# GATB/MindTheGap

Measured on AMD Instinct MI355X. Metric: breakpoints filled/sec, higher is better.
Workload: dtype u64; 1 GPU; synthetic human-scale: 3 Gbp i.i.d. donor as 600000 x 5 kb sequences, 100000 insertion sites (50-1000 nt) per batch, k=31, max-nodes 100; sites_per_batch=100000, sites_per_rank_and_step=100000, distinct_batches_per_rank=4, site_set=400000, donor_sequences=600000, erroneous_fragments=0, k=31, max_nodes=100, max_length=10000, nb_solid_kmers=3108581096, nb_unitigs=600024, index_bytes=60154587216, unitig_store_bytes=3945966160, batches_in_flight=6, input=prepared batches, resident in HBM, output=C-ABI records + ASCII sequences in page-locked host memory

## Files before the change

### mindthegap_amd/csrc/mtg_gpu_fill.hip

```cpp
#include "mtg_gpu_common.h"

namespace mtgi {

enum { TRAVERSAL_SETS = mtg_index::NWS };
__constant__ Index c_ix[TRAVERSAL_SETS];
__constant__ FillCfg c_cfg[TRAVERSAL_SETS];

#ifndef MTG_STAGE_A_WAVES
#define MTG_STAGE_A_WAVES 2
#endif
#ifndef MTG_WALK_WAVES
#define MTG_WALK_WAVES 2
#endif
enum { PARK_LISTS = 19 };
struct ParkCtl {
    uint32_t count[PARK_LISTS];
    uint32_t n_branching;
    uint32_t pad_[3];
#ifdef MTG_BUBBLE_TIMING
    uint32_t hist_lane[32], hist_wave[32], hist_walk_lane[32], hist_walk_wave[32];
#endif
};
#ifdef MTG_BUBBLE_TIMING
__device__ __forceinline__ void timing_note(uint32_t* hl, uint32_t* hw, uint64_t t0)
// ... 950 lines not shown
            const uint32_t general_hint = ws.post_general == ~0u ? m : (uint32_t)std::min<uint64_t>(m, 4ull * ws.post_general + 1024ull);
            hipLaunchKernelGGL(k_post, dim3(general_hint), dim3(64), 0, stream, idx->dev, cfg, d_raw.as<uint8_t>(), d_head.as<uint8_t>(), d_out.as<GapOut>(), ids, d_tle, d_tbad, d_toff, d_tcnt, d_mis, d_fok,
                               in.want_all_contigs ? 1u : 0u, d_rec.as<SlotRec>(), m, park, (const uint32_t*)d_pi_head, (const uint32_t*)d_pi_next, pi_mask, d_rw, d_roff, d_tie_p);
            hipLaunchKernelGGL(k_post_lean, dim3((m + 64 / POST_LEAN_G - 1) / (64 / POST_LEAN_G)), dim3(64), 0, stream, idx->dev, cfg, d_raw.as<uint8_t>(), d_head.as<uint8_t>(), d_out.as<GapOut>(), in.want_all_contigs ? 1u : 0u, d_rec.as<SlotRec>(), m);
            const ScanBegin sbegin{{0, 0, arena_used[0], arena_used[1]}};
            hipLaunchKernelGGL(k_scan1, dim3(nblocks), dim3(SCAN_SL), 0, stream, d_rec.as<SlotRec>(), m, d_blocks.as<ScanBlock>());
            hipLaunchKernelGGL(k_scan2, dim3(1), dim3(256), 0, stream, d_blocks.as<ScanBlock>(), nblocks, sbegin, d_tot.as<PartTot>(), h_tot, park);
            HIP_TRY(hipGetLastError());
            EmitDev D;
            EmitHost H;
            const double share = std::min(1.0, std::max(0.0, tune::f(tune::T_PACKED_SEQ_SHARE, 0.0)));
            const uint32_t pack_q = (uint32_t)std::lround(share * 65536.0);
            bool packed = want_records && combo && identity && arena_used[0] == 0 && pack_q != 0;
            uint64_t shadow_halves = 0;
            if (packed) {
                shadow_halves = 2 * ((((uint64_t)sink.seq_cap * pack_q) >> 16) / 32 + 3);
                HIP_TRY(d_shadow.alloc(shadow_halves * 4));
            }
            auto emit = [&]() -> int {
                D.seq = sink.seq_dev ? sink.seq_dev : p_seq(); D.ext = d_ext.as<char>();
                D.seq_cap = sink.seq_cap; D.ext_cap = sink.ext_cap;
                D.res = p_res(); D.fil = p_fil();
                D.dense_words = d_dw.as<uint64_t>(); D.dense_meta = d_dm.as<uint32_t>();
                D.dense_cap_words = ws.cap[d_dw.slot] / 8; D.dense_cap_contigs = ws.cap[d_dm.slot] / 20;
                const bool want_wire = sink.wire_dev != nullptr && identity && tier == 0;
                D.wire = want_wire ? (uint8_t*)sink.wire_dev : nullptr; D.wire_cap = sink.wire_cap; D.wire_tag = sink.wire_tag;
                D.tot = d_tot.as<PartTot>(); D.wire_gaps = m;
                D.shadow = packed ? d_shadow.as<uint32_t>() : nullptr; D.shadow_cap = shadow_halves; D.pack_q = pack_q;
                if (packed) HIP_TRY(hipMemsetAsync(d_shadow.p, 0, shadow_halves * 4, stream));
                if (want_wire) HIP_TRY(hipMemsetAsync(sink.wire_dev, 0, sizeof(mtg_wire_header), stream));
                H.seq = sink.seq; H.ext = sink.ext; H.fil = sink.fil;
                if (!want_wire)
                    hipLaunchKernelGGL(k_emit_lean, dim3((m + 64 / EMIT_LEAN_G - 1) / (64 / EMIT_LEAN_G)), dim3(64), 0, stream, idx->dev.us, cfg, d_raw.as<uint8_t>(), d_head.as<uint8_t>(), d_rec.as<SlotRec>(), d_blocks.as<ScanBlock>(),
                                       ids, d_flags, k, D, H, m);
                hipLaunchKernelGGL(k_emit, dim3(want_wire ? m : general_hint), dim3(64), 0, stream, idx->dev.us, cfg, d_raw.as<uint8_t>(), d_head.as<uint8_t>(), d_rec.as<SlotRec>(), d_blocks.as<ScanBlock>(), ids, d_flags, k, D, H,
                                   d_rlist.as<uint32_t>(), d_glist.as<uint32_t>(), m, park, want_wire ? 0u : 1u);
                if (want_wire) hipLaunchKernelGGL(k_wire_sum, dim3(256 * 4), dim3(256), 0, stream, (uint8_t*)sink.wire_dev, sink.wire_cap);
                HIP_TRY(hipGetLastError());
                return MTG_OK;
            };
            HIP_TRY(mark(eve));
            if (int erc = emit()) return erc;
            HIP_TRY(hipEventRecord(ev2, stream));
            tick("host prep+launch");
            if (while_busy && !busy_done) { busy_done = true; (*while_busy)(); tick("host work during kernels"); }
            HIP_TRY(hipEventSynchronize(ev2));
            traversal_lock.unlock();
            tick("totals ready");
            t0 = now_ms();
            PartTot tot = *h_tot;
            const uint64_t need_w = tot.end[0] * 8 + 64, need_m = tot.end[1] * 20 + 64;
            bool again = false;
            if (want_records && tot.end[2] > sink.seq_cap) {
                const uintptr_t old = (uintptr_t)sink.seq, old_end = old + sink.seq_cap;
                const uintptr_t old_fil = (uintptr_t)sink.fil, old_fil_end = old_fil + n * sizeof(mtg_filled);
                if (!sink.grow_seq || !sink.grow_seq((size_t)tot.end[2], (size_t)tot.begin[2])) { set_error("sequence buffer too small: %llu bytes needed", (unsigned long long)tot.end[2]); return MTG_ERR_ARG; }
                if (launches > 1 && (uintptr_t)sink.seq != old)
                    for (size_t i = 0; i < n; i++) { const uintptr_t q = (uintptr_t)sink.fil[i].seq; if (q >= old && q < old_end) sink.fil[i].seq = sink.seq + (q - old); }
                if (launches > 1 && (uintptr_t)sink.fil != old_fil)
                    for (size_t i = 0; i < n; i++) { const uintptr_t q = (uintptr_t)sink.res[i].filled; if (q >= old_fil && q < old_fil_end) sink.res[i].filled = (const mtg_filled*)((const char*)sink.fil + (q - old_fil)); }
                again = true;
            }
            if (want_records && tot.end[3] > sink.ext_cap) {
                const uintptr_t old = (uintptr_t)sink.ext, old_end = old + sink.ext_cap;
                if (!sink.grow_ext || !sink.grow_ext((size_t)tot.end[3], (size_t)tot.begin[3])) { set_error("extension buffer too small: %llu bytes needed", (unsigned long long)tot.end[3]); return MTG_ERR_NOMEM; }
                if (launches > 1 && (uintptr_t)sink.ext != old)
                    for (size_t i = 0; i < n; i++) { const uintptr_t q = (uintptr_t)sink.res[i].extension; if (q >= old && q < old_end) sink.res[i].extension = sink.ext + (q - old); }
                again = true;
            }
            if (need_w > ws.cap[d_dw.slot] || need_m > ws.cap[d_dm.slot]) again = true;
            if (again) {
                HIP_TRY(hipStreamSynchronize(stream));
                if (combo) HIP_TRY(d_combo.grow_keeping(sink.combo_off_seq + std::max<size_t>(sink.seq_cap, 64) + SEQ_SLACK, sink.combo_off_seq + (size_t)tot.begin[2]));
                else if (!sink.seq_dev) HIP_TRY(d_seq.grow_keeping(std::max<size_t>(sink.seq_cap, 64) + SEQ_SLACK, (size_t)tot.begin[2]));
                HIP_TRY(d_ext.alloc(std::max<size_t>(sink.ext_cap, 64)));
                HIP_TRY(d_dw.alloc(need_w));
                HIP_TRY(d_dm.alloc(need_m));
                hipLaunchKernelGGL(k_scan1, dim3(nblocks), dim3(SCAN_SL), 0, stream, d_rec.as<SlotRec>(), m, d_blocks.as<ScanBlock>());
                hipLaunchKernelGGL(k_scan2, dim3(1), dim3(256), 0, stream, d_blocks.as<ScanBlock>(), nblocks, sbegin, d_tot.as<PartTot>(), (PartTot*)nullptr, park);
                packed = false;
                if (int erc = emit()) return erc;
            }
            CopyTurn copy_turn(idx->device);
            std::vector<mtg_gap_result> tmp_res;
            std::vector<mtg_filled> tmp_fil;
            const bool one_copy = combo && identity && tot.begin[2] == 0;
            const uint64_t pack_x = packed ? packed_split(tot.end[2], pack_q) : 0, pack_words = packed ? (tot.end[2] - pack_x + 31) / 32 : 0;
            uint64_t* h_shadow = nullptr;
            if (packed) {
                h_shadow = (uint64_t*)staging_host(&ws, Workspace::NHOST - 3, pack_words * 8 + 64);
                if (!h_shadow) { set_error("no page-locked memory for the packed sequences of a launch"); return MTG_ERR_NOMEM; }
            }
            if (want_records) {
                if (h_shadow) {
                    HIP_TRY(hipMemcpyAsync(sink.combo, d_combo.p, sink.combo_off_seq, hipMemcpyDeviceToHost, stream));
                    if (pack_words) HIP_TRY(hipMemcpyAsync(h_shadow, d_shadow.p, pack_words * 8, hipMemcpyDeviceToHost, stream));
                    HIP_TRY(hipEventRecord(evp, stream));
                    if (pack_x) HIP_TRY(hipMemcpyAsync(sink.combo + sink.combo_off_seq, (const char*)d_combo.p + sink.combo_off_seq, pack_x, hipMemcpyDeviceToHost, stream));
                } else if (one_copy) HIP_TRY(hipMemcpyAsync(sink.combo, d_combo.p, sink.combo_off_seq + (size_t)tot.end[2], hipMemcpyDeviceToHost, stream));
                else if (identity) {
                    HIP_TRY(hipMemcpyAsync(sink.res, p_res(), (size_t)m * sizeof(mtg_gap_result), hipMemcpyDeviceToHost, stream));
                    HIP_TRY(hipMemcpyAsync(sink.fil, p_fil(), (size_t)m * sizeof(mtg_filled), hipMemcpyDeviceToHost, stream));
                } else {
                    tmp_res.resize(m);
                    tmp_fil.resize(m);
                    HIP_TRY(hipMemcpyAsync(tmp_res.data(), p_res(), (size_t)m * sizeof(mtg_gap_result), hipMemcpyDeviceToHost, stream));
                    HIP_TRY(hipMemcpyAsync(tmp_fil.data(), p_fil(), (size_t)m * sizeof(mtg_filled), hipMemcpyDeviceToHost, stream));
                }
                const WireLayout wl = wire_layout(m, tot.n_filled, tot.end[2], tot.end[3]);
                const bool wired = sink.wire_dev != nullptr && identity && tier == 0 && wl.total <= sink.wire_cap && tot.n_retry == 0 && tot.n_general == 0;
                if (sink.wire_dev && identity && tier == 0) { sink.wire_ok = wired; sink.wire_bytes = wired ? wl.total : 0; }
                const char* seq_src = wired ? (const char*)sink.wire_dev + wl.o_seq : (sink.seq_dev ? sink.seq_dev : p_seq());
                if (!one_copy && !sink.seq_on_device && !sink.seq_stays_in_workspace && tot.end[2] > tot.begin[2]) HIP_TRY(hipMemcpyAsync(sink.seq + tot.begin[2], seq_src + tot.begin[2], tot.end[2] - tot.begin[2], hipMemcpyDeviceToHost, stream));
                if (tot.end[3] > tot.begin[3]) HIP_TRY(hipMemcpyAsync(sink.ext + tot.begin[3], d_ext.as<char>() + tot.begin[3], tot.end[3] - tot.begin[3], hipMemcpyDeviceToHost, stream));
            }
            std::vector<uint32_t> rlist(tot.n_retry), glist(tot.n_general);
            const bool dev_general = tot.n_general > 0 && !host_paths && !in.want_all_contigs && !tune::on(tune::T_HOST_GENERAL) && !tl_host_general;
            GenCtl* h_gctl = nullptr;
            GenDev GD{};
            if (dev_general) {
                const uint64_t ng = tot.n_general;
                HIP_TRY(d_paths.alloc(ng * (size_t)PATHS_WORDS * 4));
                HIP_TRY(d_ggaps.alloc(ng * sizeof(GenGap) + sizeof(GenCtl)));
                GD.cap_sols = 4 * ng + 1024; GD.cap_ascii = ng * 1280 + (1u << 20); GD.cap_tmp = ng * 48 + (1u << 17); GD.cap_bnd = 1u << 22;
                HIP_TRY(d_gsols.alloc(GD.cap_sols * sizeof(GenSol)));
                HIP_TRY(d_gascii.alloc(GD.cap_ascii + 64));
                HIP_TRY(d_gtmp.alloc(GD.cap_tmp * 8));
                HIP_TRY(d_gbnd.alloc(GD.cap_bnd * sizeof(NwCell)));
                GD.ctl = (GenCtl*)d_ggaps.p;
                GD.gaps = (GenGap*)((char*)d_ggaps.p + sizeof(GenCtl));
                GD.sols = d_gsols.as<GenSol>(); GD.ascii = d_gascii.as<char>(); GD.tmp = d_gtmp.as<uint64_t>(); GD.bnd = d_gbnd.as<NwCell>();
                HIP_TRY(hipMemsetAsync(GD.ctl, 0, sizeof(GenCtl), stream));
                hipLaunchKernelGGL(k_paths, dim3((unsigned)ng), dim3(64), 0, stream, cfg, d_raw.as<uint8_t>(), d_head.as<uint8_t>(), d_out.as<GapOut>(), d_glist.as<uint32_t>(), k, d_paths.as<uint32_t>(), (uint32_t)ng);
                hipLaunchKernelGGL(k_general, dim3((unsigned)ng), dim3(64), 0, stream, idx->dev, cfg, d_raw.as<uint8_t>(), d_head.as<uint8_t>(), d_out.as<GapOut>(), d_glist.as<uint32_t>(), ids, d_paths.as<uint32_t>(),
                                   d_tcnt, d_fok, d_src, d_flags, k, GD, (uint32_t)ng);
                HIP_TRY(hipGetLastError());
                h_gctl = (GenCtl*)staging_host(&ws, Workspace::NHOST - 2, sizeof(GenCtl) + ng * sizeof(GenGap) + 64);
                if (!h_gctl) { set_error("no page-locked memory for the multi-contig gaps of a launch"); return MTG_ERR_NOMEM; }
                HIP_TRY(hipMemcpyAsync(h_gctl, d_ggaps.p, sizeof(GenCtl) + ng * sizeof(GenGap), hipMemcpyDeviceToHost, stream));
            }
            HostChunk* hc = nullptr;
            SlotRec* h_rec = nullptr;
            uint64_t* h_w = nullptr;
            uint32_t* h_m = nullptr;
            const uint64_t tw = tot.end[0], tc = tot.end[1];
            if (tot.n_retry) HIP_TRY(hipMemcpyAsync(rlist.data(), d_rlist.p, (size_t)tot.n_retry * 4, hipMemcpyDeviceToHost, stream));
            auto contigs_to_host = [&]() -> int {
                hc->carve(m, tw, tc, h_rec, h_w, h_m);
                HIP_TRY(hipMemcpyAsync(h_rec, d_rec.p, (size_t)m * sizeof(SlotRec), hipMemcpyDeviceToHost, stream));
                if (tw) HIP_TRY(hipMemcpyAsync(h_w, d_dw.p, tw * 8, hipMemcpyDeviceToHost, stream));
                if (tc) HIP_TRY(hipMemcpyAsync(h_m, d_dm.p, tc * 20, hipMemcpyDeviceToHost, stream));
                return MTG_OK;
            };
            if (tot.n_general) {
                special.chunks.emplace_back(new HostChunk());
                hc = special.chunks.back().get();
                HIP_TRY(hipMemcpyAsync(glist.data(), d_glist.p, (size_t)tot.n_general * 4, hipMemcpyDeviceToHost, stream));
                if (!dev_general) { if (int crc = contigs_to_host()) return crc; }
            }
            HIP_TRY(hipEventRecord(ev3, stream));
            if (h_shadow) {
                HIP_TRY(hipEventSynchronize(evp));
                const double tx = now_ms();
                expand_packed_tail(h_shadow, sink.seq, pack_x, tot.end[2], sink.res, sink.fil, n, std::min(8, std::max(1, Pool::cpu_budget() / 2)));
                if (dbg) fprintf(stderr, "  [device_run] %-18s %.3f ms (%llu of %llu arena bytes from %llu words)\n", "packed tail", now_ms() - tx,
                                 (unsigned long long)(tot.end[2] - pack_x), (unsigned long long)tot.end[2], (unsigned long long)pack_words);
            }
            HIP_TRY(hipEventSynchronize(ev3));
            copy_turn.release();
            st.d2h_ms += now_ms() - t0;
            tick("results on the host");
            t0 = now_ms();
            st.index_lines += tot.lines; st.contig_nt += tot.contig_nt; st.store_runs += tot.store_runs; st.run_nt += tot.run_nt; st.post_lines += tot.post_lines;
            st.contig_words += tot.contig_words; st.coverage_kmers += tot.cov_kmers; st.dense_words += tw;
            st.copy_words += tot.copy_words; st.copy_cmds += tot.copy_cmds; st.coverage_direct_kmers += tot.cov_direct; st.n_lean_gaps += tot.n_lean;
            if (tier == 0 && identity) ws.post_general = m - (uint32_t)std::min<uint64_t>(tot.n_lean, m);
            st.copy_words_executed += tot.copy_words_exec; st.copy_cmds_executed += tot.copy_cmds_exec; st.post_scanned_words += tot.scan_words;
            sink.seq_used = tot.end[2];
            sink.ext_used = tot.end[3];
            arena_used[0] = tot.end[2];
            arena_used[1] = tot.end[3];
            sink.n_filled += tot.n_filled;
            if (want_records && !identity)
                for (uint32_t s2 = 0; s2 < m; s2++) { sink.res[host_ids[s2]] = tmp_res[s2]; sink.fil[host_ids[s2]] = tmp_fil[s2]; }
            for (uint32_t s2 : rlist) retry.push_back(host_ids ? host_ids[s2] : s2);
            if (tot.n_retry) sink.in_gap_order = false;
            if (hc && dev_general) {
                const uint64_t ng = tot.n_general;
                const GenCtl ctl = *h_gctl;
                const GenGap* hg = (const GenGap*)(h_gctl + 1);
                hc->gen_gaps.assign(hg, hg + ng);
                uint64_t n_host = 0;
                for (uint64_t i = 0; i < ng; i++) n_host += hg[i].status != GEN_OK;
                const uint64_t ns = std::min<uint64_t>(ctl.n_sols, GD.cap_sols), na = std::min<uint64_t>(ctl.ascii_bytes, GD.cap_ascii);
                hc->gen_sols.resize(ns);
                hc->gen_ascii.resize(na + 1);
                if (ns) HIP_TRY(hipMemcpyAsync(hc->gen_sols.data(), d_gsols.p, ns * sizeof(GenSol), hipMemcpyDeviceToHost, stream));
                if (na) HIP_TRY(hipMemcpyAsync(hc->gen_ascii.data(), d_gascii.p, na, hipMemcpyDeviceToHost, stream));
                if (host_ids) hc->gap_of.assign(host_ids, host_ids + m);
                const uint32_t chunk_id = (uint32_t)special.chunks.size() - 1;
                for (uint32_t i = 0; i < (uint32_t)ng; i++) special.special.push_back(SpecialGap{host_ids ? host_ids[glist[i]] : glist[i], chunk_id, glist[i], i});
                if (n_host) {
                    if (int crc = contigs_to_host()) return crc;
                    hc->path_of.assign(m, -1);
                    if (2 * n_host > ng) {
                        hc->paths.resize(ng * (size_t)PATHS_WORDS);
                        HIP_TRY(hipMemcpyAsync(hc->paths.data(), d_paths.p, ng * (size_t)PATHS_WORDS * 4, hipMemcpyDeviceToHost, stream));
                        for (uint32_t i = 0; i < (uint32_t)ng; i++) if (hg[i].status != GEN_OK) hc->path_of[glist[i]] = (int32_t)i;
                    } else {
                        hc->paths.resize(n_host * (size_t)PATHS_WORDS);
                        uint64_t q = 0;
                        for (uint32_t i = 0; i < (uint32_t)ng; i++)
                            if (hg[i].status != GEN_OK) {
                                HIP_TRY(hipMemcpyAsync(hc->paths.data() + q * PATHS_WORDS, d_paths.as<uint32_t>() + (size_t)i * PATHS_WORDS, (size_t)PATHS_WORDS * 4, hipMemcpyDeviceToHost, stream));
                                hc->path_of[glist[i]] = (int32_t)q++;
                            }
                    }
                }
                HIP_TRY(hipStreamSynchronize(stream));
                if (n_host) h_w[tw] = 0;
                st.n_general_host += n_host;
                st.n_general_device += ng - n_host;
            } else if (hc) {
                h_w[tw] = 0;
                if (host_ids) hc->gap_of.assign(host_ids, host_ids + m);
                const uint32_t chunk_id = (uint32_t)special.chunks.size() - 1;
                std::vector<uint32_t> pslots;
                st.n_general_host += glist.size();
                uint32_t grank = 0;
                for (uint32_t s2 : glist) {
                    special.special.push_back(SpecialGap{host_ids ? host_ids[s2] : s2, chunk_id, s2, grank++});
                    if (!host_paths && !in.want_all_contigs && h_rec[s2].p.fast == 0 && h_rec[s2].p.nb_terminal > 0) pslots.push_back(s2);
                }
                if (!pslots.empty()) {
                    HIP_TRY(d_ids.alloc(std::max<size_t>(chunk, pslots.size()) * 4));
                    HIP_TRY(hipMemcpyAsync(d_ids.p, pslots.data(), pslots.size() * 4, hipMemcpyHostToDevice, stream));
                    HIP_TRY(d_paths.alloc(pslots.size() * (size_t)PATHS_WORDS * 4));
                    hipLaunchKernelGGL(k_paths, dim3((unsigned)pslots.size()), dim3(64), 0, stream, cfg, d_raw.as<uint8_t>(), d_head.as<uint8_t>(), d_out.as<GapOut>(), d_ids.as<uint32_t>(), k,
                                       d_paths.as<uint32_t>(), (uint32_t)pslots.size());
                    HIP_TRY(hipGetLastError());
                    hc->paths.resize(pslots.size() * (size_t)PATHS_WORDS);
                    HIP_TRY(hipMemcpyAsync(hc->paths.data(), d_paths.p, hc->paths.size() * 4, hipMemcpyDeviceToHost, stream));
                    HIP_TRY(hipStreamSynchronize(stream));
                    hc->path_of.assign(m, -1);
                    for (size_t g2 = 0; g2 < pslots.size(); g2++) hc->path_of[pslots[g2]] = (int32_t)g2;
                }
            }
            st.host_ms += now_ms() - t0;
            {
                const uint32_t np = tot.n_parked;
                st.n_parked_gaps += np;
                st.n_rounds += (uint64_t)rounds;
// ... 103 lines not shown
```

### mindthegap_amd/csrc/mtg_host.cpp

```cpp
#include "mtg_internal.h"
#include "mtg_dict_order.h"
#include <unistd.h>

#include <algorithm>
#include <atomic>
#include <chrono>
#include <cstdio>
#include <cstdlib>
#include <cstring>
#include <mutex>
#include <set>

extern "C" {
size_t mtg_tuning_count(void) { return (size_t)mtgi::tune::T_COUNT; }
int mtg_tuning_describe(size_t i, const char** name, const char** dflt, const char** kind, const char** what)
{
    using namespace mtgi::tune;
    if (i >= (size_t)T_COUNT) { mtgi::set_error("no tuning entry %zu", i); return MTG_ERR_ARG; }
    if (name) *name = g_entries[i].name;
    if (dflt) *dflt = g_entries[i].dflt;
    if (kind) *kind = g_entries[i].kind;
    if (what) *what = g_entries[i].what;
    return MTG_OK;
}
// ... 406 lines not shown
#if defined(__x86_64__)
__attribute__((target("bmi2"))) inline uint64_t pack32_bmi2(const char* b)
{
    uint64_t c[4];
    memcpy(c, b, 32);
    const uint64_t M = 0x0606060606060606ull;
    return _pext_u64(c[0], M) | (_pext_u64(c[1], M) << 16) | (_pext_u64(c[2], M) << 32) | (_pext_u64(c[3], M) << 48);
}
const bool have_bmi2 = __builtin_cpu_supports("bmi2") && !tune::on(tune::T_NO_VEC);
#endif
inline uint64_t pack32(const char* b)
{
#if defined(__x86_64__)
    if (have_bmi2) return pack32_bmi2(b);
#endif
    uint64_t w = 0;
    for (int i = 0; i < 32; i++) w |= (uint64_t)nt_code((unsigned char)b[i]) << (2 * i);
    return w;
}
inline void pack_lsb(const char* s, size_t n, uint64_t* out)
{
    size_t i = 0, w = 0;
    for (; i + 32 <= n; i += 32) out[w++] = pack32(s + i);
    if (i < n) {
        char b[32] = {0};
        memcpy(b, s + i, n - i);
        const size_t r = n - i;
        out[w] = pack32(b) & (r < 32 ? (1ull << (2 * r)) - 1 : ~0ull);
    }
}
inline bool all_upper_acgt(const char* s, size_t n)
{
    static const struct Tab { bool ok[256]; Tab() { memset(ok, 0, sizeof ok); ok['A'] = ok['C'] = ok['G'] = ok['T'] = true; } } tab;
    bool ok = true;
    size_t i = 0;
#if defined(__x86_64__)
    static const bool vec = !tune::on(tune::T_NO_VEC);
    if (vec) {
        const __m128i A = _mm_set1_epi8('A'), C = _mm_set1_epi8('C'), G = _mm_set1_epi8('G'), T = _mm_set1_epi8('T');
        for (; i + 16 <= n; i += 16) {
            const __m128i v = _mm_loadu_si128(reinterpret_cast<const __m128i*>(s + i));
            const __m128i m = _mm_or_si128(_mm_or_si128(_mm_cmpeq_epi8(v, A), _mm_cmpeq_epi8(v, C)), _mm_or_si128(_mm_cmpeq_epi8(v, G), _mm_cmpeq_epi8(v, T)));
            if (_mm_movemask_epi8(m) != 0xFFFF) return false;
        }
    }
#endif
    for (; i < n; i++) ok &= tab.ok[(unsigned char)s[i]];
    return ok;
}
}

void expand_codes_scalar(const uint64_t* w, size_t b, size_t e, char* out)
{
    static const char NT[4] = {'A', 'C', 'T', 'G'};
    for (size_t i = b; i < e; i++) out[i] = NT[(w[i >> 5] >> (2 * (i & 31))) & 3];
}
#if defined(__x86_64__)
__attribute__((target("avx2"))) static void expand_codes_avx2(const uint64_t* w, size_t b, size_t e, char* out)
{
    size_t i = b;
    const size_t head = std::min(e, (b + 31) & ~(size_t)31);
    expand_codes_scalar(w, i, head, out);
    i = head;
    const __m256i spread = _mm256_setr_epi8(0, 0, 0, 0, 1, 1, 1, 1, 2, 2, 2, 2, 3, 3, 3, 3, 4, 4, 4, 4, 5, 5, 5, 5, 6, 6, 6, 6, 7, 7, 7, 7);
    const __m256i field = _mm256_set1_epi32((int)0xC0300C03u), low = _mm256_set1_epi8(0x0F);
    const __m256i lut = _mm256_setr_epi8('A', 'C', 'T', 'G', 'C', 0, 0, 0, 'T', 0, 0, 0, 'G', 0, 0, 0, 'A', 'C', 'T', 'G', 'C', 0, 0, 0, 'T', 0, 0, 0, 'G', 0, 0, 0);
    for (; i + 32 <= e; i += 32) {
        __m256i t = _mm256_and_si256(_mm256_shuffle_epi8(_mm256_set1_epi64x((long long)w[i >> 5]), spread), field);
        t = _mm256_and_si256(_mm256_or_si256(t, _mm256_srli_epi16(t, 4)), low);
        _mm256_storeu_si256(reinterpret_cast<__m256i*>(out + i), _mm256_shuffle_epi8(lut, t));
    }
    expand_codes_scalar(w, i, e, out);
}
static const bool have_avx2 = __builtin_cpu_supports("avx2") && !tune::on(tune::T_NO_VEC);
#endif
void expand_codes(const uint64_t* w, size_t b, size_t e, char* out)
{
#if defined(__x86_64__)
    if (have_avx2) { expand_codes_avx2(w, b, e, out); return; }
#endif
    expand_codes_scalar(w, b, e, out);
}

void expand_packed_tail(const uint64_t* w, char* seq, uint64_t x, uint64_t end, const mtg_gap_result* res, const mtg_filled* fil, size_t n, int nthreads)
{
    if (end <= x || n == 0) return;
    const size_t pieces = std::min<size_t>(n, 256);
    auto first_fill = [&](size_t g, size_t lim) { while (g < lim && res[g].n_filled == 0) g++; return g; };
    auto start_of = [&](size_t g) { return (uint64_t)(fil[g].seq - seq); };
    parallel_for(pieces, nthreads, [&](size_t c) {
        const size_t g0 = n * c / pieces, g1 = n * (c + 1) / pieces;
        const size_t f = first_fill(g0, g1);
        if (f == g1) return;
        const size_t nf = first_fill(g1, n);
        const uint64_t lo = std::max<uint64_t>(start_of(f), x), hi = std::min<uint64_t>(nf < n ? start_of(nf) : end, end);
        if (hi <= lo) return;
        expand_codes(w, lo - x, hi - x, seq + x);
        for (size_t g = f + 1; g < g1; g++) {
            if (res[g].n_filled == 0) continue;
            const uint64_t z = start_of(g) - 1;
            if (z >= lo && z < hi) seq[z] = 0;
        }
        seq[hi - 1] = 0;
    }, 1);
}

void FillInput::set_common(size_t g, std::string_view source, std::string_view swf_target, int nb_mis, uint8_t gap_flags)
{
    flags[g] = gap_flags;
    const uint64_t kfields = kmask(k);
    char sb[32] = {0};
    memcpy(sb, source.data(), (size_t)k);
    const uint64_t sp = pack32(sb) & kfields;
    src[g] = reverse_fields(sp) >> (64 - 2 * k);
    const size_t rl = swf_target.size(), w0 = roff[g];
    const size_t nw = (rl + 31) / 32 + 1;
    rwords[w0 + nw - 1] = 0;
    if (nw >= 2) rwords[w0 + nw - 2] = 0;
    pack_lsb(swf_target.data(), rl, rwords.p + w0);
    r0[g] = rl >= (size_t)k ? reverse_fields(rwords[w0] & kfields) >> (64 - 2 * k) : 0;
    if (!all_upper_acgt(swf_target.data(), rl)) { rlen[g] = 0xFFFFFFFFu; r0[g] = 0; }
    nbmis[g] = (uint8_t)nb_mis;
    bool ok = (int)source.size() == k;
    if (ok) {
        uint64_t c[4];
        memcpy(c, sb, 32);
        ok = ((c[0] | c[1] | c[2] | c[3]) & 0x0808080808080808ull) == 0;
    }
    fast_ok[g] = ok ? 1 : 0;
}
void FillInput::set_target(size_t o, std::string_view seq)
{
    uint8_t* slot = traw.p + o * TARGET_SLOT;
    const bool usable = (int)seq.size() >= k;
    memset(slot, 0, TARGET_SLOT);
    if (usable) memcpy(slot, seq.data(), (size_t)k);
    slot[TARGET_SLOT - 1] = usable ? 1 : 0;
}
struct ContigGraph {
    std::vector<std::vector<int>> in_edges;
    ContigGraph(const GapDev& gc, int k)
    {
        const uint32_t n = gc.o.n_contigs;
        in_edges.resize(n);
        const uint64_t mk1 = kmask(k - 1);
        auto kmer_at = [&](uint32_t c, uint32_t start) {
            const uint64_t* w = gc.words + gc.word_start[c];
            uint64_t f = 0;
            for (int j = 0; j < k - 1; j++) { uint32_t i = start + j; f = (f << 2) | ((w[i >> 5] >> (2 * (i & 31))) & 3ull); }
            return f & mk1;
        };
        std::unordered_map<uint64_t, std::vector<int>> by_prefix;
        for (uint32_t j = 0; j < n; j++) by_prefix[kmer_at(j, 0)].push_back((int)j);
        for (uint32_t i = 0; i < n; i++) {
            auto it = by_prefix.find(kmer_at(i, gc.len[i] - (k - 1)));
            if (it == by_prefix.end()) continue;
            for (int j : it->second) {
                if (j == (int)i && (int)gc.len[i] == k - 1) continue;
                in_edges[j].push_back((int)i);
            }
        }
        for (auto& v : in_edges) { std::sort(v.begin(), v.end()); v.erase(std::unique(v.begin(), v.end()), v.end()); }
    }
};

typedef std::vector<int> Path;
typedef std::set<std::pair<Path, int>> PathSet;

struct RevDfs {
    const ContigGraph& g;
    const std::vector<TermInfo>& terms;
    int terminal_node, target;
    int nb_calls = 0;
    bool success = true;
    static const size_t max_breadth = 20;
    std::set<Path> run(int start_node, const Path& current)
    {
        std::set<Path> paths;
        if (nb_calls++ > 10000000) { success = false; return paths; }
        if (start_node != terminal_node)
            for (auto& t : terms) if (t.node == start_node) return paths;
        if (start_node == 0) { paths.insert(current); return paths; }
        for (int next : g.in_edges[start_node]) {
            if (std::find(current.begin(), current.end(), next) == current.end()) {
                Path ext;
                ext.reserve(current.size() + 1);
                ext.push_back(next);
// ... 1564 lines not shown
```

### mindthegap_amd/csrc/mtg_internal.h

```cpp
#ifndef MTG_INTERNAL_H
#define MTG_INTERNAL_H
#include "../../include/mtg_fill.h"
#include "mtg_hostutil.h"
#include "mtg_paths.h"
#include "mtg_general.h"
#include "mtg_emit.h"
#include "mtg_copy.h"
#include "mtg_format.h"
#include "mtg_tuning.h"
#include <algorithm>
#include <atomic>
#include <condition_variable>
#include <cstdio>
#include <cstdlib>
#include <cstring>
#include <functional>
#include <memory>
#include <mutex>
#include <sched.h>
#include <string>
#include <string_view>
#include <thread>
#include <vector>

// ... 138 lines not shown
            bool mine = false;
            for (int spin = 0; spin < SPIN && !mine; spin++) {
                if (stop_.load(std::memory_order_relaxed)) return;
                const uint64_t g = gen_.load(std::memory_order_acquire);
                if (g != seen) { seen = g; mine = claim(); }
                else cpu_relax();
            }
            if (!mine) {
                std::unique_lock<std::mutex> lk(m_);
                cv_.wait(lk, [&] { return stop_.load() || gen_.load(std::memory_order_acquire) != seen; });
                if (stop_.load()) return;
                seen = gen_.load(std::memory_order_acquire);
                mine = claim();
            }
            if (!mine) continue;
            (*job_)();
            if (active_.fetch_sub(1, std::memory_order_acq_rel) == 1) {
                std::lock_guard<std::mutex> lk(m_);
                done_cv_.notify_all();
            }
        }
    }
    std::vector<std::thread> threads_;
    std::mutex m_, run_mtx_;
    std::condition_variable cv_, done_cv_;
    const std::function<void()>* job_ = nullptr;
    std::atomic<int> to_start_{0}, active_{0};
    std::atomic<uint64_t> gen_{0};
    std::atomic<bool> stop_{false};
};

template <typename F> inline void parallel_for(size_t n, int nthreads, F f, size_t grain = 64)
{
    if (nthreads <= 0) nthreads = Pool::get().size();
    if ((size_t)nthreads * grain > n) nthreads = (int)std::max<size_t>(n / grain, 1);
    if (nthreads <= 1) { for (size_t i = 0; i < n; i++) f(i); return; }
    std::atomic<size_t> next{0};
    std::function<void()> work = [&]() {
        for (;;) {
            const size_t b = next.fetch_add(grain);
            if (b >= n) break;
            const size_t e = std::min(n, b + grain);
            for (size_t i = b; i < e; i++) f(i);
        }
    };
    Pool::get().run(nthreads, work);
}

template <typename G> inline uint64_t parallel_prefix(size_t n, int nthreads, uint64_t* out, G get)
{
    const size_t B = 4096, nb = (n + B - 1) / B;
    std::vector<uint64_t> bs(nb + 1, 0);
    out[0] = 0;
    parallel_for(nb, nthreads, [&](size_t b) {
        uint64_t sum = 0;
        for (size_t i = b * B; i < std::min(n, (b + 1) * B); i++) { const uint64_t v = get(i); out[i + 1] = v; sum += v; }
        bs[b + 1] = sum;
    }, 1);
    for (size_t b = 0; b < nb; b++) bs[b + 1] += bs[b];
    parallel_for(nb, nthreads, [&](size_t b) {
        uint64_t run = bs[b];
        for (size_t i = b * B; i < std::min(n, (b + 1) * B); i++) { run += out[i + 1]; out[i + 1] = run; }
    }, 1);
    return bs[nb];
}

struct Target {
    std::string_view seq, name;
    bool is_rc = false;
};
struct TargetSpan {
    const Target* p = nullptr;
    uint32_t n = 0;
    size_t size() const { return n; }
    const Target& operator[](size_t i) const { return p[i]; }
    const Target* begin() const { return p; }
    const Target* end() const { return p + n; }
};

void* staging_host(Workspace* ws, int slot, size_t bytes);
void expand_codes(const uint64_t* w, size_t b, size_t e, char* out);
void expand_codes_scalar(const uint64_t* w, size_t b, size_t e, char* out);
void expand_packed_tail(const uint64_t* w, char* seq, uint64_t x, uint64_t end, const mtg_gap_result* res, const mtg_filled* fil, size_t n, int nthreads);
void* pinned_alloc(size_t bytes);
void pinned_free(void* p);
int host_register(void* p, size_t bytes);
int host_unregister(void* p);
int device_download(const mtg_index* idx, void* host_dst, const void* dev_src, size_t bytes);
int device_upload(const mtg_index* idx, void* dev_dst, const void* host_src, size_t bytes);

template <typename T> struct Arr {
    T* p = nullptr;
    size_t n = 0;
    T* data() const { return p; }
    size_t size() const { return n; }
    bool empty() const { return n == 0; }
    T& operator[](size_t i) const { return p[i]; }
};
struct FillInput {
    int k = 31;
    bool want_all_contigs = false;
    Workspace* ws = nullptr;
    Arr<uint64_t> src;
    Arr<uint64_t> r0;
    Arr<uint32_t> roff;
    Arr<uint32_t> rlen;
    Arr<uint32_t> toff, tcnt;
    Arr<uint8_t> nbmis, fast_ok, flags;
    Arr<uint64_t> rwords;
    Arr<uint8_t> traw;
    void *block_a = nullptr, *block_b = nullptr, *block_c = nullptr;
    size_t bytes_a = 0, bytes_b = 0, bytes_c = 0;
    std::vector<uint64_t> own_a, own_b, own_c;
    void* dev_a = nullptr; void* dev_b = nullptr; void* dev_tenc = nullptr;
    bool text_mode = false;
    uint64_t n_rwords = 0, n_text_targets = 0, text_bytes = 0;
    const char* text_direct = nullptr;
    struct Shared {
        const uint64_t* enc = nullptr;
        uint32_t n = 0;
        const uint32_t* pi = nullptr;
        uint32_t pi_mask = 0;
    } shared;
    uint8_t* tie_out = nullptr;
    static size_t text_block_off(size_t n, size_t nt, int which)
    {
        const size_t o[6] = {0, 8 * n, 16 * n, 16 * n + 8 * nt, 20 * n + 8 * nt, (20 * n + 12 * nt + 7) & ~(size_t)7};
        return o[which];
    }
    void resize(size_t n);
    void size(size_t i, size_t swf_len, size_t n_targets) { rlen[i] = (uint32_t)swf_len; tcnt[i] = (uint32_t)n_targets; }
    void layout();
    void set_common(size_t i, std::string_view source, std::string_view swf_target, int nb_mis, uint8_t gap_flags);
    void set_target(size_t slot, std::string_view seq);
    enum { BLOCK = 512 };
    std::vector<uint64_t> blk_rw, blk_nt;
    std::vector<uint32_t> slen;
    void alloc_b(uint64_t rw, uint64_t nt);
    template <typename SizeFn> void plan(size_t n, int nthreads, SizeFn sz)
    {
        resize(n);
        slen.resize(n);
        const size_t nb = (n + BLOCK - 1) / BLOCK;
        blk_rw.assign(nb + 1, 0);
        blk_nt.assign(nb + 1, 0);
        parallel_for(nb, nthreads, [&](size_t b) {
            uint64_t rw = 0, nt = 0;
            for (size_t i = b * BLOCK; i < std::min(n, (b + 1) * (size_t)BLOCK); i++) {
                size_t sl = 0, tn = 0;
                sz(i, sl, tn);
                size(i, sl, tn);
                rw += (sl + 31) / 32 + 1;
                nt += tn;
            }
            blk_rw[b + 1] = rw;
            blk_nt[b + 1] = nt;
        }, 1);
        for (size_t b = 0; b < nb; b++) { blk_rw[b + 1] += blk_rw[b]; blk_nt[b + 1] += blk_nt[b]; }
        alloc_b(blk_rw[nb], blk_nt[nb]);
    }
    template <typename SizeFn, typename SetFn> bool plan_and_fill(size_t n, int nthreads, SizeFn sz, SetFn st)
    {
        resize(n);
        slen.resize(n);
        const size_t nb = (n + BLOCK - 1) / BLOCK;
        blk_rw.assign(nb + 1, 0);
// ... 268 lines not shown
```

### mindthegap_amd/csrc/mtg_tuning.h

```cpp
#ifndef MTG_TUNING_H
#define MTG_TUNING_H
#include <stddef.h>
#include <stdio.h>
#include <stdlib.h>
#include <string.h>
#include <mutex>
#include <string>

#define MTG_TUNABLES(X) \
    X(POOL_THREADS, "", "cap", "size of the host worker pool (default: the CPUs the process may use -- hardware threads, affinity mask, cgroup quota -- at most 64); read when the pool starts") \
    X(PACKED_SEQ_SHARE, "0.75", "cap", "share (0..1) of a whole-batch launch's sequence arena that crosses the link 2-bit packed, the host expanding it to ASCII (0: every byte as ASCII)") \
    X(COPY_SLOTS, "3", "cap", "batches of a device that copy their results to the host at the same time (0: no limit); more copies at once share the link worse") \
    X(UPLOAD_OWN_STREAM, "", "ab", "every batch uploads its input on its own stream instead of the device's one upload stream (three uploads at a time take the link from the downloads: profiles/r04_text_entry.txt)") \
    X(SPARSE_ADJ_LOAD, "0.49", "cap", "load factor of the sparse junction table, as a share of the dense one's; 0.7 overflows the displacement range at human scale") \
    X(JT_LOAD, "0.7", "cap", "load factor of the lean build's junction table") \
    X(BLOOM_BITS, "12", "cap", "Bloom filter bits per k-mer (0: no filter, no sequence scan)") \
    X(LOAD_THREADS, "", "cap", "threads that stream a container's abundance bytes to the device (default: up to 8)") \
    X(LOAD_PIECE, "", "test", "k-mers per piece when an index container is loaded (default 2^26): small pieces exercise the piece loop") \
    X(COUNT_PASSES, "", "test", "force this many passes of the k-mer counting (default: as many as HBM needs)") \
    X(ROUNDS, "", "ab", "bubble rounds between launches of the walk kernel (default: 6 when most gaps of the previous launch parked, else 0)") \
    X(LIGHT_WALK, "", "ab", "1 / 0: the first walk of a launch by the light kernel (simple paths only, every branching node parks) / by the full one; default: light when fewer than 1 in 128 gaps of the previous launch met a branching node") \
    X(BUILD_PARTITIONED, "", "ab", "the junction table of packed sequences built partition by partition in LDS (1) or by scattered insertion (0); default: partitioned from 2^27 junction positions on") \
    X(NO_SPLIT_LONG, "", "test", "index construction from packed sequences: a sequence of more than 131 072 nucleotides stays one work item (no pieces of 65 536 that share k - 1 nucleotides)") \
    X(BUILD_POSITIONAL, "", "ab", "packed sequences: the chains that lie whole in one sequence are found by position (1, default) or every chain is walked on the junction table (0)") \
    X(FINISH_G, "", "ab", "lanes per parked gap in the finishing kernel: 1, 8, 16 or 64 (default: 64 while few gaps park, 16 otherwise)") \
    X(FINISH_WAVE_BELOW, "2048", "ab", "a whole wave per parked gap while the previous launch parked fewer gaps than this") \
    X(NO_POST_INDEX, "", "test", "the terminal search counts every contig position against every target of its gap (no piece index of the batch's dictionaries)") \
    X(NO_LEAN, "", "test", "every contig is materialised (no lean gaps)") \
    X(NO_DEFER, "", "test", "the lanes of the traversal copy their long runs themselves (no copy commands, no k_copy work)") \
    X(MAX_CHUNK, "", "test", "gaps per traversal launch (default: what the scratch holds): several launches per batch") \
    X(HOST_GENERAL, "", "test", "the multi-contig gaps by the host's path (candidate sequences, de-duplication, coverage: as until round 4) instead of k_general") \
    X(HOST_PATHS, "", "test", "leave the path enumeration of multi-contig gaps to the host") \
    X(DEBUG_SKIP_FINISH, "", "diag", "parked gaps stay parked (and fail as overflowing gaps)") \
    X(KERNEL_TIMERS, "", "diag", "every batch records an event between its kernels and mtg_last_batch_stats carries each kernel's own time (off: three events per batch instead of nine, only device_span_ms)") \
    X(DEBUG_TIMERS, "", "diag", "per-phase wall times of every batch and every index construction on stderr") \
    X(NO_VEC, "", "test", "scalar instead of vector host code (pext in the input pass, AVX2 in the expansion of a packed arena)") \
    X(NO_PREFETCH, "", "test", "no software prefetch in the input pass") \
    X(NB_GPUS, "", "cap", "the tool: devices to use (default: all visible; -nb-gpus overrides)") \
    X(CLI_BATCH, "", "cap", "the tool: sites per batch (default 100 000)") \
    X(CLI_IN_FLIGHT, "", "cap", "the tool: worker threads per device (default 3, at most 6)") \
    X(CLI_WRITERS, "1", "cap", "the tool: writer threads per output file (a file's lock serialises write(2): more than one per file was measured the same or slower)") \
    X(CLI_NO_MMAP, "", "test", "the tool reads its breakpoint file instead of mapping it") \
    X(CONTIG_PER_SEED, "", "ab", "contig mode (the tool and mtg_fill_seeds): every seed gets its own copy of the dictionary (mtg_fill_batch, as until round 6) instead of the shared table on the device") \
    X(HOST_FORMAT, "", "ab", "the tool: every site's text by the host's writers (round 3) instead of the device's formatter") \
    X(TOOL_TIMERS, "", "diag", "the tool: where the time of a run went (stderr)") \
    X(TOOL_QUIET, "", "diag", "the tool: no summary on stdout")

namespace mtgi {
namespace tune {
enum Id {
#define MTG_TUNE_ENUM(name, dflt, kind, what) T_##name,
    MTG_TUNABLES(MTG_TUNE_ENUM)
#undef MTG_TUNE_ENUM
    T_COUNT
};
struct Entry { const char* name; const char* env; const char* dflt; const char* kind; const char* what; };
inline const Entry g_entries[T_COUNT] = {
#define MTG_TUNE_ROW(name, dflt, kind, what) {#name, "MTG_" #name, dflt, kind, what},
    MTG_TUNABLES(MTG_TUNE_ROW)
#undef MTG_TUNE_ROW
};
struct Values {
    std::mutex m;
    char v[T_COUNT][64];
    bool forced[T_COUNT];
    Values()
    {
        memset(v, 0, sizeof v);
        memset(forced, 0, sizeof forced);
        if (const char* e = getenv("MTG_TUNING")) {
            std::string all(e);
            size_t b = 0;
            while (b < all.size()) {
                size_t c = all.find(',', b);
                if (c == std::string::npos) c = all.size();
                const std::string item = all.substr(b, c - b);
                const size_t eq = item.find('=');
                const std::string nm = item.substr(0, eq), val = eq == std::string::npos ? "1" : item.substr(eq + 1);
                const int t = find(nm.c_str());
                if (t >= 0) put(t, val.c_str());
                else fprintf(stderr, "MTG_TUNING: no entry named %s (mtg_tuning_describe lists them)\n", nm.c_str());
                b = c + 1;
            }
        }
    }
    static int find(const char* name)
    {
        if (!name) return -1;
        if (!strncmp(name, "MTG_", 4)) name += 4;
        for (int t = 0; t < T_COUNT; t++) if (!strcmp(g_entries[t].name, name)) return t;
        return -1;
    }
    bool put(int t, const char* val)
    {
// ... 30 lines not shown
```

Before: 233.7 million breakpoints/s.

## Expand packed sequence tail on a persistent crew, overlapping with the copy turn

Replaces the blocking parallel_for expansion of the 2-bit packed sequence tail with a persistent host thread crew. Work is split into fixed-size byte pieces sized to fit L2, and the batch submits these pieces before waiting for the remaining device-to-host copies. The copy turn is therefore released while expansion is still running, and the calling thread joins in only afterwards. This trades extra spinning threads and a more complex synchronisation path for overlap between the host-side expansion and the DMA, and for better load balance.

```diff
diff --git a/mindthegap_amd/csrc/mtg_gpu_fill.hip b/mindthegap_amd/csrc/mtg_gpu_fill.hip
--- a/mindthegap_amd/csrc/mtg_gpu_fill.hip
+++ b/mindthegap_amd/csrc/mtg_gpu_fill.hip
@@ -1056,6 +1056,7 @@
                 if (int erc = emit()) return erc;
             }
             CopyTurn copy_turn(idx->device);
+            const double t_turn = now_ms();
             std::vector<mtg_gap_result> tmp_res;
             std::vector<mtg_filled> tmp_fil;
             const bool one_copy = combo && identity && tot.begin[2] == 0;
@@ -1133,15 +1134,23 @@
                 if (!dev_general) { if (int crc = contigs_to_host()) return crc; }
             }
             HIP_TRY(hipEventRecord(ev3, stream));
+            ExpandBatch expansion;
+            double tx = 0;
             if (h_shadow) {
                 HIP_TRY(hipEventSynchronize(evp));
-                const double tx = now_ms();
-                expand_packed_tail(h_shadow, sink.seq, pack_x, tot.end[2], sink.res, sink.fil, n, std::min(8, std::max(1, Pool::cpu_budget() / 2)));
-                if (dbg) fprintf(stderr, "  [device_run] %-18s %.3f ms (%llu of %llu arena bytes from %llu words)\n", "packed tail", now_ms() - tx,
-                                 (unsigned long long)(tot.end[2] - pack_x), (unsigned long long)tot.end[2], (unsigned long long)pack_words);
+                tx = now_ms();
+                const int crew = tune::is_set(tune::T_EXPAND_THREADS) ? (int)tune::i(tune::T_EXPAND_THREADS) : std::min(8, std::max(1, Pool::cpu_budget() / 2));
+                expansion.submit(h_shadow, sink.seq, pack_x, tot.end[2], sink.res, sink.fil, n, crew);
             }
             HIP_TRY(hipEventSynchronize(ev3));
             copy_turn.release();
+            if (h_shadow) {
+                const double t_rel = now_ms();
+                expansion.finish();
+                if (dbg) fprintf(stderr, "  [device_run] %-18s %.3f ms (%llu of %llu arena bytes from %llu words; last piece %.3f ms after the shadow arrived, copy turn held %.3f ms, %u of %u pieces on this thread)\n",
+                                 "packed tail", now_ms() - t_rel, (unsigned long long)(tot.end[2] - pack_x), (unsigned long long)tot.end[2], (unsigned long long)pack_words, now_ms() - tx, t_rel - t_turn,
+                                 expansion.ran_here(), expansion.pieces());
+            }
             st.d2h_ms += now_ms() - t0;
             tick("results on the host");
             t0 = now_ms();
diff --git a/mindthegap_amd/csrc/mtg_host.cpp b/mindthegap_amd/csrc/mtg_host.cpp
--- a/mindthegap_amd/csrc/mtg_host.cpp
+++ b/mindthegap_amd/csrc/mtg_host.cpp
@@ -512,27 +512,166 @@
     expand_codes_scalar(w, b, e, out);
 }
 
+namespace {
+void expand_piece(const ExpandBatch& b, uint32_t c)
+{
+    enum { BLOCK = 4096 };
+    const uint64_t lo = b.x + (uint64_t)c * b.piece, hi = std::min(b.end, lo + b.piece);
+    const size_t n = b.n;
+    auto first_fill = [&](size_t g, size_t lim) { while (g < lim && b.res[g].n_filled == 0) g++; return g; };
+    auto start_of = [&](size_t g) { return (uint64_t)(b.fil[g].seq - b.seq); };
+    size_t ga = 0, gb = n;
+    while (ga < gb) {
+        const size_t mid = ga + (gb - ga) / 2, f = first_fill(mid, gb);
+        if (f == gb || start_of(f) > lo) gb = mid;
+        else ga = f + 1;
+    }
+    size_t g = first_fill(ga, n);
+    for (uint64_t p = lo; p < hi;) {
+        const uint64_t q = std::min<uint64_t>(hi, p + BLOCK);
+        char* out = b.seq + p;
+        expand_codes(b.w + (p - b.x) / 32, 0, q - p, out);
+        for (; g < n; g = first_fill(g + 1, n)) {
+            const uint64_t z = start_of(g) - 1;
+            if (z >= q) break;
+            if (z >= p) out[z - p] = 0;
+        }
+        if (q == b.end) out[q - 1 - p] = 0;
+        p = q;
+    }
+}
+
+class Expander {
+public:
+    static Expander& get() { static Expander e; return e; }
+    void submit(ExpandBatch& b, int crew)
+    {
+        int wake = 0;
+        bool all = false, waiters = false;
+        {
+            std::lock_guard<std::mutex> lk(m_);
+            const int want = std::max(0, std::min<int>(crew, MAX_CREW));
+            try {
+                while ((int)threads_.size() < want) { const int i = (int)threads_.size(); threads_.emplace_back([this, i] { loop(i); }); }
+            } catch (const std::system_error&) {}
+            limit_.store(want, std::memory_order_relaxed);
+            b.link = nullptr;
+            if (tail_) tail_->link = &b; else head_ = &b;
+            tail_ = &b;
+            queued_.fetch_add(b.npieces, std::memory_order_release);
+            all = want < (int)threads_.size();
+            wake = (int)std::min<uint32_t>(b.npieces, (uint32_t)sleepers_);
+            waiters = waiters_ > 0;
+        }
+        if (all) { if (wake) work_cv_.notify_all(); }
+        else for (int i = 0; i < wake; i++) work_cv_.notify_one();
+        if (waiters) done_cv_.notify_all();
+    }
+    void finish(ExpandBatch& b)
+    {
+        for (;;) {
+            if (b.pending.load(std::memory_order_acquire) == 0) return;
+            ExpandBatch* t = nullptr;
+            uint32_t c = 0;
+            if (take(t, c)) {
+                if (t == &b) b.own++;
+                run(t, c);
+                continue;
+            }
+            bool again = false;
+            for (int spin = 0; spin < SPIN && !again; spin++) {
+                again = b.pending.load(std::memory_order_acquire) == 0 || queued_.load(std::memory_order_acquire) != 0;
+                if (!again) Pool::cpu_relax();
+            }
+            if (again) continue;
+            std::unique_lock<std::mutex> lk(m_);
+            waiters_++;
+            done_cv_.wait(lk, [&] { return b.pending.load(std::memory_order_acquire) == 0 || head_ != nullptr; });
+            waiters_--;
+        }
+    }
+
+private:
+    enum { SPIN = 2000, MAX_CREW = 64 };
+    Expander() {}
+    ~Expander()
+    {
+        { std::lock_guard<std::mutex> lk(m_); stop_.store(true); }
+        work_cv_.notify_all();
+        for (auto& t : threads_) t.join();
+    }
+    bool take(ExpandBatch*& b, uint32_t& c)
+    {
+        std::lock_guard<std::mutex> lk(m_);
+        if (!head_) return false;
+        b = head_;
+        c = b->next++;
+        if (b->next == b->npieces) { head_ = b->link; if (!head_) tail_ = nullptr; }
+        queued_.fetch_sub(1, std::memory_order_relaxed);
+        return true;
+    }
+    void run(ExpandBatch* b, uint32_t c)
+    {
+        expand_piece(*b, c);
+        if (b->pending.fetch_sub(1, std::memory_order_acq_rel) == 1) {
+            std::lock_guard<std::mutex> lk(m_);
+            if (waiters_) done_cv_.notify_all();
+        }
+    }
+    void loop(int i)
+    {
+        for (;;) {
+            ExpandBatch* b = nullptr;
+            uint32_t c = 0;
+            bool mine = false;
+            for (int spin = 0; spin < SPIN && !mine; spin++) {
+                if (stop_.load(std::memory_order_relaxed)) return;
+                if (i < limit_.load(std::memory_order_relaxed) && queued_.load(std::memory_order_acquire) != 0) mine = take(b, c);
+                else Pool::cpu_relax();
+            }
+            if (!mine) {
+                std::unique_lock<std::mutex> lk(m_);
+                sleepers_++;
+                work_cv_.wait(lk, [&] { return stop_.load() || (i < limit_.load(std::memory_order_relaxed) && head_ != nullptr); });
+                sleepers_--;
+                if (stop_.load()) return;
+                continue;
+            }
+            run(b, c);
+        }
+    }
+    std::mutex m_;
+    std::condition_variable work_cv_, done_cv_;
+    ExpandBatch *head_ = nullptr, *tail_ = nullptr;
+    std::vector<std::thread> threads_;
+    int sleepers_ = 0, waiters_ = 0;
+    std::atomic<uint64_t> queued_{0};
+    std::atomic<int> limit_{0};
+    std::atomic<bool> stop_{false};
+};
+}
+
+void ExpandBatch::submit(const uint64_t* w_, char* seq_, uint64_t x_, uint64_t end_, const mtg_gap_result* res_, const mtg_filled* fil_, size_t n_, int crew)
+{
+    finish();
+    if (end_ <= x_ || n_ == 0) return;
+    w = w_; seq = seq_; x = x_; end = end_; res = res_; fil = fil_; n = n_;
+    piece = (uint64_t)std::max<long>(32, tune::i(tune::T_EXPAND_PIECE, 262144) & ~31L);
+    npieces = (uint32_t)((end - x + piece - 1) / piece);
+    next = 0; own = 0;
+    pending.store(npieces, std::memory_order_relaxed);
+    Expander::get().submit(*this, crew);
+}
+void ExpandBatch::finish()
+{
+    if (pending.load(std::memory_order_acquire) != 0) Expander::get().finish(*this);
+}
+
 void expand_packed_tail(const uint64_t* w, char* seq, uint64_t x, uint64_t end, const mtg_gap_result* res, const mtg_filled* fil, size_t n, int nthreads)
 {
-    if (end <= x || n == 0) return;
-    const size_t pieces = std::min<size_t>(n, 256);
-    auto first_fill = [&](size_t g, size_t lim) { while (g < lim && res[g].n_filled == 0) g++; return g; };
-    auto start_of = [&](size_t g) { return (uint64_t)(fil[g].seq - seq); };
-    parallel_for(pieces, nthreads, [&](size_t c) {
-        const size_t g0 = n * c / pieces, g1 = n * (c + 1) / pieces;
-        const size_t f = first_fill(g0, g1);
-        if (f == g1) return;
-        const size_t nf = first_fill(g1, n);
-        const uint64_t lo = std::max<uint64_t>(start_of(f), x), hi = std::min<uint64_t>(nf < n ? start_of(nf) : end, end);
-        if (hi <= lo) return;
-        expand_codes(w, lo - x, hi - x, seq + x);
-        for (size_t g = f + 1; g < g1; g++) {
-            if (res[g].n_filled == 0) continue;
-            const uint64_t z = start_of(g) - 1;
-            if (z >= lo && z < hi) seq[z] = 0;
-        }
-        seq[hi - 1] = 0;
-    }, 1);
+    ExpandBatch b;
+    b.submit(w, seq, x, end, res, fil, n, nthreads - 1);
+    b.finish();
 }
 
 void FillInput::set_common(size_t g, std::string_view source, std::string_view swf_target, int nb_mis, uint8_t gap_flags)
diff --git a/mindthegap_amd/csrc/mtg_internal.h b/mindthegap_amd/csrc/mtg_internal.h
--- a/mindthegap_amd/csrc/mtg_internal.h
+++ b/mindthegap_amd/csrc/mtg_internal.h
@@ -244,6 +244,25 @@
 void expand_codes(const uint64_t* w, size_t b, size_t e, char* out);
 void expand_codes_scalar(const uint64_t* w, size_t b, size_t e, char* out);
 void expand_packed_tail(const uint64_t* w, char* seq, uint64_t x, uint64_t end, const mtg_gap_result* res, const mtg_filled* fil, size_t n, int nthreads);
+struct ExpandBatch {
+    ExpandBatch() {}
+    ExpandBatch(const ExpandBatch&) = delete;
+    ExpandBatch& operator=(const ExpandBatch&) = delete;
+    ~ExpandBatch() { finish(); }
+    void submit(const uint64_t* w, char* seq, uint64_t x, uint64_t end, const mtg_gap_result* res, const mtg_filled* fil, size_t n, int crew);
+    void finish();
+    uint32_t pieces() const { return npieces; }
+    uint32_t ran_here() const { return own; }
+    const uint64_t* w = nullptr;
+    char* seq = nullptr;
+    uint64_t x = 0, end = 0, piece = 0;
+    const mtg_gap_result* res = nullptr;
+    const mtg_filled* fil = nullptr;
+    size_t n = 0;
+    uint32_t npieces = 0, next = 0, own = 0;
+    std::atomic<uint32_t> pending{0};
+    ExpandBatch* link = nullptr;
+};
 void* pinned_alloc(size_t bytes);
 void pinned_free(void* p);
 int host_register(void* p, size_t bytes);
diff --git a/mindthegap_amd/csrc/mtg_tuning.h b/mindthegap_amd/csrc/mtg_tuning.h
--- a/mindthegap_amd/csrc/mtg_tuning.h
+++ b/mindthegap_amd/csrc/mtg_tuning.h
@@ -10,6 +10,8 @@
 #define MTG_TUNABLES(X) \
     X(POOL_THREADS, "", "cap", "size of the host worker pool (default: the CPUs the process may use -- hardware threads, affinity mask, cgroup quota -- at most 64); read when the pool starts") \
     X(PACKED_SEQ_SHARE, "0.75", "cap", "share (0..1) of a whole-batch launch's sequence arena that crosses the link 2-bit packed, the host expanding it to ASCII (0: every byte as ASCII)") \
+    X(EXPAND_THREADS, "", "cap", "threads of the crew that expands packed sequence arenas next to the batches' own threads (default: half the CPUs the process may use, 1 to 8; 0: no crew, the batches' threads do all of it)") \
+    X(EXPAND_PIECE, "262144", "cap", "arena bytes one piece of that expansion writes (rounded down to a multiple of 32, at least 32): its output and its codes should fit a core's L2") \
     X(COPY_SLOTS, "3", "cap", "batches of a device that copy their results to the host at the same time (0: no limit); more copies at once share the link worse") \
     X(UPLOAD_OWN_STREAM, "", "ab", "every batch uploads its input on its own stream instead of the device's one upload stream (three uploads at a time take the link from the downloads: profiles/r04_text_entry.txt)") \
     X(SPARSE_ADJ_LOAD, "0.49", "cap", "load factor of the sparse junction table, as a share of the dense one's; 0.7 overflows the displacement range at human scale") \
```

Result: slower. 213.4 million breakpoints/s (-8.6%).
